# cwozny/sdr_channelizer

Hardware: AMD Instinct MI355X
Metric: input MS/s (complex) channelized (higher is better)
Workload: dtype f32; 1 GPU; cfg2: M=64 channels, 12 taps/branch, D=64, int16 I/Q (12-bit), 2^30 samples per GPU per step, frame-major complex64 out; kernel=pfb_fast<M64,P12,D64,int16>, schedule=default (4: FIR/FFT wave pairs, 8x64-frame workgroups), samples_per_gpu=1073741824, prewarm_steps=20, parallelism=single GPU

## Files before the change

### sdr_channelizer_amd/csrc/pfb_api.cpp

```cpp
#include <hip/hip_runtime.h>

#include <algorithm>
#include <cmath>
#include <cstdio>
#include <cstring>
#include <new>
#include <stdexcept>
#include <string>
#include <utility>
#include <vector>

#include "pfb_common.h"
#include "pfb_channelizer_dev.h"
#include "pfb_host.h"
#include "pfb_launch_policy.h"

using pfb::DeviceGuard;
using pfb::g_detail;
using pfb::hip_fail;

namespace {

constexpr uint32_t kStateMagic = 0x50464231u;

struct StateHeader {
  uint32_t magic, M, P, D, fmt, hist_samples, phase, reserved;
  uint64_t frame_index;
};

}

struct pfb_handle {
  int M = 0, P = 0, D = 0, off = 0;
  int fmt = 0, bit_width = 0, layout = 0;
  unsigned flags = 0;
  int device = 0;
  int num_cus = 256;
  int bps = 0;
// ... 95 lines not shown
    q.layout = PFB_LAYOUT_FRAME_MAJOR;
    q.out = static_cast<float2*>(h->d_slab);
    q.frames = std::min<long long>(sf, p.frames - f0);
    q.frame0 = p.frame0 + f0;
    q.in = static_cast<const char*>(p.in) + (size_t)f0 * h->D * h->bps;
    q.n_in = p.n_in - f0 * h->D;
    if (f0 > 0)
      q.hist = static_cast<const char*>(q.in) - (size_t)h->hist_samples * h->bps;
    HIP_TRY(h->fast->launch(q, h->stream));
    HIP_TRY(pfb::launch_transpose_slab(h->d_slab, q.frames, h->M, p.out, p.out_ld, p.out_frame0 + f0, h->out_elem, h->stream));
  }
  return PFB_OK;
}

int launch_frames(pfb_handle* h, const void* d_iq, uint64_t n, const void* hist, void* d_out, uint64_t f_begin,
                  uint64_t f_end, int64_t out_ld, int64_t out_frame0) {
  if (f_end <= f_begin) return PFB_OK;
  if (f_begin > 0) {
    if (f_begin * (uint64_t)h->D < (uint64_t)h->hist_samples) return PFB_ERR_BAD_ARG;
    const size_t skip = (size_t)f_begin * h->D * h->bps;
    hist = static_cast<const char*>(d_iq) + skip - (size_t)h->hist_samples * h->bps;
    d_iq = static_cast<const char*>(d_iq) + skip;
    n -= f_begin * (uint64_t)h->D;
    if (h->layout == PFB_LAYOUT_FRAME_MAJOR) d_out = static_cast<char*>(d_out) + (size_t)f_begin * h->M * h->out_elem;
    else out_frame0 += (int64_t)f_begin;
  }
  const uint64_t frames = f_end - f_begin;
  pfb::KernelParams p{};
  p.in = d_iq;
  p.hist = hist;
  p.out = static_cast<float2*>(d_out);
// ... 24 lines not shown
  if (prc != PFB_OK) return prc;
  if (want_fast) {
    const pfb::LaunchRequest rq{h->opt_schedule, h->opt_frames_per_block, h->opt_xcd_remap, h->opt_slab_frames,
                                h->layout == PFB_LAYOUT_CHANNEL_MAJOR, (h->flags & PFB_FLAG_MAGNITUDE) != 0, h->num_cus};
    const pfb_launch_report rep = pfb::plan_launch(h->plan, rq, frames);
    p.schedule = rep.schedule;
    p.frames_per_block = rep.frames_per_block;
    p.xcd_remap = rep.xcd_remap;
    const int cpt = h->fast->cols_per_thread;
    const int bmod = ((p.base % cpt) + cpt) % cpt;
    p.vec_ok = (bmod == 0) && (reinterpret_cast<uintptr_t>(d_iq) % (uintptr_t)(h->bps * cpt) == 0);
    if (rep.by_slabs) {
      const int rc = launch_by_slabs(h, p, (long long)rep.slab_frames);
      if (rc != PFB_OK) return rc;
    } else {
      HIP_TRY(h->fast->launch(p, h->stream));
    }
    h->last_kernel = h->fast->name;
    h->last_launch = rep;
  } else {
    HIP_TRY(pfb::launch_generic(p, h->stream));
    h->last_kernel = "pfb_generic";
    h->last_launch = pfb_launch_report{};
    h->last_launch.frames = frames;
  }
  if (ev_second) HIP_TRY(hipEventRecord(ev_second, h->stream));
  return PFB_OK;
}

int advance_state(pfb_handle* h, const void* d_iq, uint64_t n, uint64_t frames) {
  if (n > 0) {
    HIP_TRY(pfb::launch_update_history(h->d_hist[h->cur], d_iq, (long long)n, h->d_hist[h->cur ^ 1],
                                       h->hist_samples, h->bps, h->stream));
    h->cur ^= 1;
  }
  h->phase = (uint32_t)((h->phase + n) % (uint64_t)h->D);
  h->frame_index += frames;
  return PFB_OK;
}

int enqueue(pfb_handle* h, const void* d_iq, uint64_t n, void* d_out, uint64_t frames, int64_t out_ld,
            int64_t out_frame0) {
  const int rc = launch_frames(h, d_iq, n, h->d_hist[h->cur], d_out, 0, frames, out_ld, out_frame0);
  if (rc != PFB_OK) return rc;
  return advance_state(h, d_iq, n, frames);
}

int process_host(pfb_handle* h, const void* iq, uint64_t n, const pfb::StageOut& out, uint64_t chunk = 0) {
  if (chunk == 0) chunk = h->opt_host_chunk > 0 ? (uint64_t)h->opt_host_chunk : (uint64_t)1 << 24;
  chunk = ((chunk + h->D - 1) / h->D) * h->D;
  const pfb::StageSteps steps{
      chunk, chunk / h->D + 1, (size_t)h->bps, (size_t)h->M * h->out_elem,
      [h](uint64_t m) { return frames_for(h, m); },
      [h](const void* d_in, uint64_t m, void* d_out, uint64_t f, int64_t out_ld, int64_t out_row0) {
        return enqueue(h, d_in, m, d_out, f, out_ld, out_row0);
      }};
  return pfb::stage_host(h->stage, h->stream, steps, iq, n, out);
}

hipError_t make_lane_tables(const pfb_handle* h, const pfb::FastKernelInfo* f, float** taps_lane, float2** tw_lane) {
// ... 742 lines not shown
```

### sdr_channelizer_amd/csrc/pfb_common.h

```cpp
#pragma once

#include <hip/hip_runtime.h>
#include <stdint.h>

#include <new>

#include "pfb_channelizer.h"

namespace pfb {

template <class F>
static inline int abi_guard(F&& body) noexcept {
  try {
    return body();
  } catch (const std::bad_alloc&) {
    return PFB_ERR_NO_MEMORY;
  } catch (...) {
    return PFB_ERR_INTERNAL;
  }
}

struct KernelParams {
  const void* in;
  const void* hist;
// ... 9 lines not shown
  long long out_frame0;
  int base;
  int hist_samples;
  int frames_per_block;
  int vec_ok;
  int M, P, D;
  int fmt;
  int layout;
  unsigned flags;
  int nontemporal;
  int xcd_remap;
  int experiment;
  int schedule;
  int tile_waves;
  int grid_override;
};

template <int FMT> struct SampleT;
template <> struct SampleT<PFB_FMT_INT16_IQ> {
  using raw_t = uint32_t;
  static constexpr int kBytes = 4;
  static __device__ __forceinline__ void cvt(raw_t v, float& re, float& im) {
    re = (float)(int16_t)(v & 0xffffu);
    im = (float)((int32_t)v >> 16);
  }
};
template <> struct SampleT<PFB_FMT_INT8_IQ> {
  using raw_t = uint16_t;
  static constexpr int kBytes = 2;
  static __device__ __forceinline__ void cvt(raw_t v, float& re, float& im) {
// ... 77 lines not shown
```

### sdr_channelizer_amd/csrc/pfb_fast.hpp

```cpp
#pragma once

#include "pfb_fast_halo.hpp"
#include "pfb_fast_overlap.hpp"
#include "pfb_fast_pairs.hpp"
#include "pfb_fast_seg.hpp"
#include "pfb_fast_sliding.hpp"
#include "pfb_fast_teams.hpp"
#include "pfb_fast_tiles.hpp"
#include "pfb_fast_twin.hpp"

namespace pfb {

template <class K>
constexpr bool kChannelMajorOk = K::NT < 1024 && !(K::NP == 3 && K::C <= 4);

template <class K>
hipError_t launch_fast(const KernelParams& p, hipStream_t s) {
  if (p.frames <= 0) return hipSuccess;
  if (p.layout == PFB_LAYOUT_CHANNEL_MAJOR) {
    if constexpr (kChannelMajorOk<K>) {
      if constexpr (K::NT == 64) {
        if constexpr (kTileTOk<K, 4, 2>) {
          if (p.schedule == 8 || p.schedule < 0) {
            const int key = p.tile_waves * 100 + (p.schedule == 8 ? p.frames_per_block / K::C : 0);
// ... 16 lines not shown
            if (nwv == 16) return launch_tile<K, 16, true>(p, s);
          }
          return launch_tile<K, 8, true>(p, s);
        }
      }
      return launch_sliding<K, true>(p, s);
    } else {
      return hipErrorInvalidValue;
    }
  }
  if constexpr (K::NT == 64 && K::NP == 2 && !K::PINGPONG) {
    if (p.schedule == 7) {
      constexpr size_t kPair = sizeof(float2) * 2 * K::BUF;
      if (p.tile_waves == 4) return launch_pairs_sliding<K, 4, 2>(p, s);
      if constexpr (K::MIN_WAVES >= 4 && 8 * kPair <= 160 * 1024) {
        if (p.tile_waves >= 8) return launch_pairs_sliding<K, 8, 4>(p, s);
      }
      return launch_pairs_sliding<K, 6, 3>(p, s);
    }
  }
  if constexpr (kOverlapOk<K>) {
    if (p.schedule == 11) return launch_overlap<K>(p, s);
  }
  if constexpr (kTwinOk<K>) {
    if (p.schedule == 13) {
      if (p.layout != PFB_LAYOUT_FRAME_MAJOR) return hipErrorInvalidValue;
      return launch_twin<K>(p, s);
    }
  }
  if constexpr (kTeamsOk<K>) {
    if (p.schedule == 6) return launch_teams<K>(p, s);
  }
  if constexpr (K::NT == 64 && K::NP == 2 && !K::PINGPONG && K::M == 64 && K::C == 8) {
    if (p.schedule == 4) {
      const int key = p.tile_waves * 1000 + p.frames_per_block;
      if constexpr (K::FMT == PFB_FMT_INT16_IQ && K::M == 64 && K::P == 12) {
        switch (key) {
          case 4064: return launch_paired<K, 4, 64, 4>(p, s);
          case 5064: return launch_paired<K, 5, 64, 5>(p, s);
          case 8048: return launch_paired<K, 8, 48, 4>(p, s);
          case 8128: return launch_paired<K, 8, 128, 4>(p, s);
          default: break;
        }
      }
      constexpr size_t kPair = sizeof(float2) * 2 * K::BUF, kSlot = sizeof(typename SampleT<K::FMT>::raw_t) * (K::W - 1) * K::D;
      if constexpr (8 * kPair + 9 * kSlot <= 160 * 1024) {
        if (p.tile_waves == 4) return launch_paired<K, 4, 64, 2>(p, s);
        return launch_paired<K, 8, 64, 4>(p, s);
      } else {
        return launch_paired<K, 4, 64, 2>(p, s);
      }
    }
  }
  if constexpr (K::NT == 64 && K::C == 8 && !K::PINGPONG) {
    if (p.schedule == 3) {
      const int key = p.tile_waves * 1000 + p.frames_per_block;
      hipError_t r = hipErrorNotSupported;
      if (key == 8024) r = launch_shared<K, 8, 24>(p, s);
      else if (key == 8032) r = launch_shared<K, 8, 32>(p, s);
      else if (key == 8064) r = launch_shared<K, 8, 64>(p, s);
      else if (key == 4064) r = launch_shared<K, 4, 64>(p, s);
      else {
        bool done = false;
        if constexpr (K::FMT == PFB_FMT_INT16_IQ && K::M == 64 && K::P == 12) {
          switch (key) {
// ... 25 lines not shown
```

### sdr_channelizer_amd/csrc/pfb_fast_cfg.hpp

```cpp
#pragma once

#include "pfb_cplx.hpp"

namespace pfb {


template <int M_, int P_, int D_, int CPT_, int FMT_, int C_, int NP_, int R0_, int R1_, int R2_, int RS0_,
          int RS1_, int RS2_, int FS_, bool PINGPONG_, int MIN_WAVES_, bool TW_TABLE_ = false, bool WAVE_FRAMES_ = false>
struct FastCfg {
  static constexpr bool WAVE_FRAMES = WAVE_FRAMES_;
  static constexpr int M = M_, P = P_, D = D_, CPT = CPT_, FMT = FMT_, C = C_, NP = NP_;
  static constexpr int LANES = D / CPT;
  static constexpr int NT = (LANES + 63) / 64 * 64;
  static constexpr bool POW2 = (M & (M - 1)) == 0;
  static constexpr int W = M * P / D;
  static constexpr int OS = M / D;
  static constexpr int FS = FS_;
  static constexpr bool PINGPONG = PINGPONG_;
  static constexpr bool TW_TABLE = TW_TABLE_;
  static constexpr int MIN_WAVES = MIN_WAVES_;
  static constexpr int R(int i) { return i == 0 ? R0_ : i == 1 ? R1_ : R2_; }
  static constexpr int RS(int i) { return i == 0 ? RS0_ : i == 1 ? RS1_ : RS2_; }
  static constexpr int S(int i) { int s = 1; for (int j = i + 1; j < NP; ++j) s *= R(j); return s; }
  static constexpr int K(int i) { int k = 1; for (int j = 0; j < i; ++j) k *= R(j); return k; }
// ... 17 lines not shown
PFB_DEV long long xcd_remap_block(long long blk, long long nb, int mode) {
  if (mode == 1) {
    const long long q = nb >> 3, r = nb & 7, xc = blk & 7;
    return (xc < r ? xc * (q + 1) : r * (q + 1) + (xc - r) * q) + (blk >> 3);
  }
  if (mode > 1) {
    const long long G = mode, span = 8 * G, base = (blk / span) * span;
    if (base + span <= nb) {
      const long long in = blk - base;
      return base + (in & 7) * G + (in >> 3);
    }
  }
  return blk;
}

template <class K>
struct FastRows {
  using ST = SampleT<K::FMT>;
  using raw_t = typename ST::raw_t;
  static constexpr int D = K::D, CPT = K::CPT, C = K::C, NT = K::NT;

  struct alignas(sizeof(raw_t) * CPT) RawVec { raw_t v[CPT]; };

  PFB_DEV v2f cvt(raw_t r) {
    float re, im;
    ST::cvt(r, re, im);
    return (v2f){re, im};
  }

  template <bool INTERIOR>
// ... 120 lines not shown
```

### sdr_channelizer_amd/csrc/pfb_fast_core.hpp

```cpp
#pragma once

#include "pfb_fast_cfg.hpp"

namespace pfb {

template <class K, bool CM = false, bool MS = false>
struct FastKernel : FastRows<K> {
  static constexpr int M = K::M, P = K::P, D = K::D, CPT = K::CPT, C = K::C, W = K::W, OS = K::OS, NT = K::NT;
  static constexpr int NW = W - 1 + C;

  template <int I, bool FULL = false, int MAGSEL = -1>
  PFB_DEV void pass(const KernelParams& p, float2* src, float2* dst, int tid, long long f0,
                    const v2f (&tw)[2][16]) {
    float2* const p_out = p.out;
    const long long p_frames = p.frames;
    constexpr int R = K::R(I), S = K::S(I), KK = K::K(I), RS = K::RS(I);
    constexpr int IPF = M / R, ITEMS = C * IPF, ITERS = (ITEMS + NT - 1) / NT;
    constexpr bool LAST = (I == K::NP - 1);
    constexpr bool TW_REGS = (ITERS == 1) && !K::TW_TABLE;
    constexpr bool READ_BARRIER = !LAST && !K::PINGPONG && NT > 64;
    constexpr bool kMagStaged = MS && LAST;
#pragma unroll
    for (int it = 0; it < ITERS; ++it) {
      const int w = tid + it * NT;
      const bool active = (ITEMS % NT == 0) || (w < ITEMS);
      const int fc = w / IPF, item = w % IPF;
      const int kk = item / S, rest = item % S;
      v2f x[R];
      if (active) {
        const v2f* s2 = reinterpret_cast<const v2f*>(src) + fc * K::FS + item;
// ... 61 lines not shown
          const int shift = (p.flags & PFB_FLAG_FFTSHIFT) ? (M / 2) : 0;
          auto col_of = [&](int ch) {
            const int c2 = ch + shift;
            return c2 >= M ? c2 - M : c2;
          };
          auto slot = [&](auto* rowp, int k) {
            if constexpr (K::POW2) {
              auto* lo = rowp + kk + shift;
              auto* hi = rowp + kk + (M / 2 - shift);
              return (k < R / 2) ? lo + k * KK : hi + (k - R / 2) * KK;
            } else {
              return rowp + col_of(kk + k * KK);
            }
          };
          if constexpr (CM || (!K::POW2 && K::NT == 64)) {
            const bool mag = (p.flags & PFB_FLAG_MAGNITUDE) != 0;
            const long long esz = mag ? 4 : 8;
            const long long cs = CM ? p.out_ld : 1;
            int col = col_of(kk);
            char* ptr = reinterpret_cast<char*>(p_out) + ((long long)col * cs + (CM ? p.out_frame0 + f : f * M)) * esz;
            const long long step = (long long)KK * cs * esz, wrap = (long long)M * cs * esz;
#pragma unroll
            for (int k = 0; k < R; ++k) {
              v2f v = x[k];
              if (mag) {
                *reinterpret_cast<float*>(ptr) = mag_out(v.x, v.y, p.flags);
              } else {
                v = derot(v, k);
                store_c64(reinterpret_cast<float2*>(ptr), v, p.nontemporal);
              }
              asm volatile("" : "+v"(ptr) : : "memory");
              col += KK;
              ptr += step;
              if (col >= M) { col -= M; ptr -= wrap; }
            }
          } else if (MAGSEL == 1 || (MAGSEL < 0 && (p.flags & PFB_FLAG_MAGNITUDE))) {
            float* rowm = reinterpret_cast<float*>(p_out) + f0 * M + fc * M;
#pragma unroll
            for (int k = 0; k < R; ++k) *slot(rowm, k) = mag_out(x[k].x, x[k].y, p.flags);
          } else {
            float2* row = p_out + f0 * M + fc * M;
#pragma unroll
            for (int k = 0; k < R; ++k) {
              const v2f v = derot(x[k], k);
              store_c64(slot(row, k), v, p.nontemporal);
            }
          }
        }
      }
    }
  }

  PFB_DEV int tslot_frame(int col, int fc) {
    constexpr int IPF = M / K::R(K::NP - 1), NFC = IPF >= 16 ? 1 : 16 / IPF, Q = 16 / C;
    static_assert(16 % C == 0 && (IPF >= 16 || 16 % IPF == 0) && C % NFC == 0, "power-of-two chunk and lane groups");
    return fc ^ (NFC * ((col / Q) % (C / NFC)));
  }

  PFB_DEV void last_pass_transposed(const KernelParams& p, float2* slot, int tid, long long f0) {
    constexpr int I = K::NP - 1;
// ... 175 lines not shown
          for (int t = 0; t < C; ++t) {
            if (q == 0 && (j & 1)) fma_tap0_hi(acc[t], x[W - 1 + t - j][cc], k.hp[j >> 1][cc]);
            else if (q == 0) fma_tap0_lo(acc[t], x[W - 1 + t - j][cc], k.hp[j >> 1][cc]);
            else if (j & 1) fma_tap_hi(acc[t], x[W - 1 + t - j][cc], k.hp[j >> 1][cc], tok);
            else fma_tap_lo(acc[t], x[W - 1 + t - j][cc], k.hp[j >> 1][cc], tok);
          }
        }
        if (!(K::LANES < NT) || tid < K::LANES) {
#pragma unroll
          for (int t = 0; t < C; ++t)
            reinterpret_cast<v2f*>(buf)[t * K::FS + k.upos[ph][cc]] = acc[t] * k.conj_mul;
        }
      }
  }

  PFB_DEV void fft_from_lds(const KernelParams& p, const Consts& k, float2* buf, int tid, long long f0) {
    static_assert(K::NP == 2 && !K::PINGPONG, "two in-place passes");
    pass<0>(p, buf, buf, tid, f0, k.tw);
    team_sync<true>();
    pass<1>(p, buf, nullptr, tid, f0, k.tw);
  }
};

}
```

### sdr_channelizer_amd/csrc/pfb_fast_halo.hpp

```cpp
#pragma once

#include "pfb_fast_core.hpp"

namespace pfb {

template <class K>
struct HaloShare : FastKernel<K> {
  using F = FastKernel<K>;
  using typename F::raw_t; using typename F::Consts;
  using F::cvt; using F::setup; using F::fir_to_lds; using F::fft_from_lds;
  static constexpr int M = K::M, P = K::P, D = K::D, CPT = K::CPT, C = K::C, W = K::W, OS = K::OS, NT = K::NT, NW = F::NW;

  template <bool INTERIOR, int NWV, int L>
  PFB_DEV void shared_impl(const KernelParams& p, const Consts& k, float2* lds, raw_t* halo_mine,
                           const raw_t* halo_next, int wave, long long f_begin) {
    static_assert(L % C == 0 && L >= W - 1, "runs are whole chunks and at least one halo long");
    constexpr int TAIL0 = L - (W - 1);
    const int tid = threadIdx.x & 63;
    const int c0 = tid * CPT;
    const raw_t* run_ptr = static_cast<const raw_t*>(p.in) + ((f_begin - (W - 1)) * D + p.base);
    v2f x[NW][CPT];
    raw_t raw[C][CPT];
#pragma unroll
    for (int i = 0; i < W - 1; ++i) {
// ... 106 lines not shown
#pragma unroll
          for (int cc = 0; cc < CPT; ++cc) x[W - 1 + t][cc] = cvt(raw[ci % DEPTH][t][cc]);
        }
      }
      if (ci + DEPTH < NCH) fetch(ci + DEPTH);
      fir_to_lds(k, x, bufs + (ci & 1) * K::BUF, tid);
#pragma unroll
      for (int i = 0; i < W - 1; ++i)
#pragma unroll
        for (int cc = 0; cc < CPT; ++cc) x[i][cc] = x[i + C][cc];
      __syncthreads();
    }
    __syncthreads();
  }

  template <int NPAIR, int L>
  PFB_DEV void run_paired(const KernelParams& p, float2* lds_fft, raw_t* lds_halo) {
    static_assert(NT == 64, "one wave per run and role");
    static_assert(L % C == 0 && L >= W - 1, "runs are whole chunks and at least one halo long");
    constexpr int NCH = L / C;
    const int wave = threadIdx.x >> 6, tid = threadIdx.x & 63;
    const bool fir_role = wave < NPAIR;
    const int pair = fir_role ? wave : wave - NPAIR;
    long long blk = blockIdx.x;
    blk = xcd_remap_block(blk, gridDim.x, p.xcd_remap);
    const long long f_blk = blk * (long long)(NPAIR * L);
    const long long f_begin = f_blk + (long long)pair * L;
    float2* bufs = lds_fft + pair * 2 * K::BUF;
    const bool interior = p.vec_ok && ((f_blk - (W - 1)) * D + p.base >= 0) && (f_blk + NPAIR * L <= p.frames);
    if (fir_role) {
      raw_t* halo_mine = lds_halo + pair * ((W - 1) * D);
      const raw_t* halo_next = lds_halo + (pair + 1) * ((W - 1) * D);
      if (interior) paired_fir_role<true, NPAIR, L>(p, bufs, halo_mine, halo_next, pair, f_begin);
      else paired_fir_role<false, NPAIR, L>(p, bufs, halo_mine, halo_next, pair, f_begin);
    } else {
      Consts k;
      setup(p, tid, k);
      __syncthreads();
#pragma unroll
      for (int s = 0; s <= NCH; ++s) {
        if (s >= 1) fft_from_lds(p, k, bufs + ((s - 1) & 1) * K::BUF, tid, f_begin + (long long)(s - 1) * C);
        __syncthreads();
      }
    }
  }
};

template <class K, int NWV, int L>
__global__ void __launch_bounds__(64 * NWV) pfb_shared_kernel(const KernelParams p) {
  using raw_t = typename SampleT<K::FMT>::raw_t;
  __shared__ float2 lds_fft[NWV * K::LDS_ELEMS];
  __shared__ raw_t lds_halo[(NWV + 1) * (K::W - 1) * K::D];
  HaloShare<K>::template run_shared<NWV, L>(p, lds_fft, lds_halo);
}

template <class K, int NPAIR, int L, int MINW>
__global__ void __launch_bounds__(128 * NPAIR, MINW) pfb_paired_kernel(const KernelParams p) {
  using raw_t = typename SampleT<K::FMT>::raw_t;
  __shared__ float2 lds_fft[NPAIR * 2 * K::BUF];
  __shared__ raw_t lds_halo[(NPAIR + 1) * (K::W - 1) * K::D];
  HaloShare<K>::template run_paired<NPAIR, L>(p, lds_fft, lds_halo);
}

template <class K, int NPAIR, int L, int MINW>
hipError_t launch_paired(const KernelParams& p, hipStream_t s) {
  return launch_blocks(&pfb_paired_kernel<K, NPAIR, L, MINW>, blocks_for(p, (long long)NPAIR * L), 128 * NPAIR, p, s);
}

template <class K, int NWV>
constexpr bool kSharedFits = sizeof(float2) * NWV * K::LDS_ELEMS +
                                 sizeof(typename SampleT<K::FMT>::raw_t) * (NWV + 1) * (K::W - 1) * K::D <= 160 * 1024;

template <class K, int NWV, int L>
hipError_t launch_shared_impl(const KernelParams& p, hipStream_t s) {
  const unsigned extra_lds = (unsigned)((p.experiment >> 8) & 0xff) * 1024u;
  return launch_blocks(&pfb_shared_kernel<K, NWV, L>, blocks_for(p, (long long)NWV * L), 64 * NWV, p, s, extra_lds);
}

template <class K, int NWV, int L>
hipError_t launch_shared(const KernelParams& p, hipStream_t s) {
  if constexpr (kSharedFits<K, NWV>) {
// ... 10 lines not shown
```

### sdr_channelizer_amd/csrc/pfb_fast_overlap.hpp

```cpp
#pragma once

#include "pfb_fast_core.hpp"
#include <utility>

namespace pfb {

template <class K>
struct Overlap : FastKernel<K> {
  using F = FastKernel<K>;
  using typename F::raw_t; using typename F::Consts;
  using F::cvt; using F::setup;
  static constexpr int M = K::M, P = K::P, D = K::D, CPT = K::CPT, C = K::C, W = K::W, OS = K::OS, NT = K::NT, NW = F::NW;

  static constexpr int NWP = (NW + C - 1) / C * C, PERIOD = NWP / C;
  static constexpr bool kRingOk = PERIOD >= 2 && PERIOD <= 4;
  static constexpr bool kBuiltinFir = OS == 2 && CPT == 1;
  template <int PH = 0, int NX = NW>
  PFB_DEV void fir_compute(const Consts& k, const v2f (&xw)[NX][CPT], v2f (&acc)[OS][CPT][C]) {
    auto x = [&](int i) -> const v2f (&)[CPT] { return xw[(i + C * PH) % NX]; };
#pragma unroll
    for (int ph = 0; ph < OS; ++ph)
#pragma unroll
      for (int cc = 0; cc < CPT; ++cc) {
        if constexpr (kBuiltinFir) {
// ... 156 lines not shown
    setup(p, threadIdx.x, k);
    const bool interior = p.vec_ok && ((f_begin - (W - 1)) * D + p.base >= 0) && (f_last <= p.frames);
    if constexpr (kRingOk) {
      if (interior && p.frames_per_block == C * PERIOD) {
        run_overlap_ring<MAGSEL>(p, k, lds, f_begin);
        return;
      }
    }
    if (interior) run_overlap_impl<true, MAGSEL>(p, k, lds, f_begin, f_end);
    else run_overlap_impl<false, MAGSEL>(p, k, lds, f_begin, f_end);
  }
};

template <class K, bool MAG>
__global__ void __launch_bounds__(K::NT, (K::MIN_WAVES > 2 ? K::MIN_WAVES - 1 : K::MIN_WAVES)) pfb_overlap_kernel(const KernelParams p) {
  __shared__ float2 lds[2 * K::BUF];
  Overlap<K>::template run_overlap<MAG ? 1 : 0>(p, lds);
}

template <class K>
constexpr bool kOverlapOk = K::NT == 64 && K::NP == 2 && !K::PINGPONG;

template <class K>
hipError_t launch_overlap(const KernelParams& p, hipStream_t s) {
  return launch_blocks(wants_magnitude(p) ? &pfb_overlap_kernel<K, true> : &pfb_overlap_kernel<K, false>,
                       blocks_for(p, p.frames_per_block), K::NT, p, s);
}

}
```

### sdr_channelizer_amd/csrc/pfb_fast_pairs.hpp

```cpp
#pragma once

#include "pfb_fast_core.hpp"

namespace pfb {

template <class K>
struct PairSlide : FastKernel<K> {
  using F = FastKernel<K>;
  using typename F::raw_t; using typename F::Consts; using typename F::RowFetch;
  using F::cvt; using F::setup; using F::finish_rows; using F::fir_to_lds; using F::fft_from_lds;
  static constexpr int M = K::M, P = K::P, D = K::D, CPT = K::CPT, C = K::C, W = K::W, OS = K::OS, NT = K::NT, NW = F::NW;

  template <bool INTERIOR>
  PFB_DEV void pair_fir_run(const KernelParams& p, const Consts& k, float2* bufs, long long f_begin, int nch) {
    const int tid = threadIdx.x & 63;
    const int c0 = tid * CPT;
    const raw_t* run_ptr = static_cast<const raw_t*>(p.in) + ((f_begin - (W - 1)) * D + p.base);
    v2f x[NW][CPT];
    raw_t raw[C][CPT];
#pragma unroll
    for (int i = 0; i < W - 1; ++i) {
      raw_t t[CPT];
      F::template load_row<INTERIOR>(p, run_ptr, f_begin - (W - 1) + i, i, c0, t);
#pragma unroll
// ... 14 lines not shown
        if (ci + 1 < nch) {
          const long long rel = (long long)(ci + 1) * C + (W - 1);
          F::template load_rows<INTERIOR>(p, run_ptr, f_begin + (long long)(ci + 1) * C, rel, c0, raw, rf);
        }
        fir_to_lds(k, x, bufs + u * K::BUF, tid);
#pragma unroll
        for (int i = 0; i < W - 1; ++i)
#pragma unroll
          for (int cc = 0; cc < CPT; ++cc) x[i][cc] = x[i + C][cc];
        __syncthreads();
      }
    }
    __syncthreads();
  }

  template <int NPAIR>
  PFB_DEV void run_pairs_sliding(const KernelParams& p, float2* lds_fft) {
    static_assert(NT == 64 && K::NP == 2 && !K::PINGPONG, "one wave per role, two in-place passes");
    const int wave = threadIdx.x >> 6, tid = threadIdx.x & 63;
    const bool fir_role = wave < NPAIR;
    const int pair = fir_role ? wave : wave - NPAIR;
    long long blk = blockIdx.x;
    blk = xcd_remap_block(blk, gridDim.x, p.xcd_remap);
    const long long f_begin = (blk * NPAIR + pair) * (long long)p.frames_per_block;
    const int nch = p.frames_per_block / C;
    float2* bufs = lds_fft + pair * 2 * K::BUF;
    Consts k;
    setup(p, tid, k);
    if (fir_role) {
      const bool interior = p.vec_ok && ((f_begin - (W - 1)) * D + p.base >= 0) && (f_begin + p.frames_per_block <= p.frames);
      if (f_begin >= p.frames) {
        for (int s = 0; s <= nch; ++s) __syncthreads();
      } else if (interior) {
        pair_fir_run<true>(p, k, bufs, f_begin, nch);
      } else {
        pair_fir_run<false>(p, k, bufs, f_begin, nch);
      }
    } else {
#pragma unroll 1
      for (int s = 0; s <= nch; ++s) {
        if (s >= 1 && f_begin < p.frames) fft_from_lds(p, k, bufs + ((s - 1) & 1) * K::BUF, tid, f_begin + (long long)(s - 1) * C);
        __syncthreads();
      }
    }
  }
};

template <class K, int NPAIR, int MINW>
__global__ void __launch_bounds__(128 * NPAIR, MINW) pfb_pairs_sliding_kernel(const KernelParams p) {
  __shared__ float2 lds_fft[NPAIR * 2 * K::BUF];
  PairSlide<K>::template run_pairs_sliding<NPAIR>(p, lds_fft);
}

template <class K, int NPAIR, int MINW>
hipError_t launch_pairs_sliding(const KernelParams& p, hipStream_t s) {
  return launch_blocks(&pfb_pairs_sliding_kernel<K, NPAIR, MINW>, blocks_for(p, (long long)NPAIR * p.frames_per_block), 128 * NPAIR, p, s);
}

}
```

### sdr_channelizer_amd/csrc/pfb_fast_seg.hpp

```cpp
#pragma once

#include "pfb_fast_cfg.hpp"

namespace pfb {

template <class K>
struct SegKernel {
  using ST = SampleT<K::FMT>;
  using raw_t = typename ST::raw_t;
  static constexpr int M = K::M, P = K::P, D = K::D, C = K::C, W = K::W;
  static constexpr int SEG = 64 / M, CT = C * SEG, NW = W - 1 + C;
  static_assert(K::NT == 64 && K::CPT == 1 && K::OS == 1 && K::NP == 2 && K::PINGPONG && SEG >= 1, "small banks");

  PFB_DEV v2f cvt(raw_t r) {
    float re, im;
    ST::cvt(r, re, im);
    return (v2f){re, im};
  }

  template <bool INTERIOR>
  PFB_DEV raw_t load(const KernelParams& p, long long s, long long f) {
    const raw_t* in = static_cast<const raw_t*>(p.in);
    if constexpr (INTERIOR) {
      return in[s];
// ... 132 lines not shown
  template <int MAGSEL = -1, int CMSEL = -1>
  PFB_DEV void run(const KernelParams& p, float2* lds) {
    long long run = blockIdx.x;
    run = xcd_remap_block(run, gridDim.x, p.xcd_remap);
    const long long f_begin = run * p.frames_per_block;
    if (f_begin >= p.frames) return;
    const long long l_seg = p.frames_per_block / SEG;
    const bool interior = p.vec_ok && ((f_begin - (W - 1)) * D + p.base >= 0) && (f_begin + p.frames_per_block <= p.frames);
    if (interior) run_impl<true, MAGSEL, CMSEL>(p, lds, f_begin, l_seg);
    else run_impl<false, MAGSEL, CMSEL>(p, lds, f_begin, l_seg);
  }
};

template <class K, bool MAG, bool CMAJ>
__global__ void __launch_bounds__(64, K::MIN_WAVES) pfb_seg_kernel(const KernelParams p) {
  __shared__ float2 lds[2 * SegKernel<K>::CT * K::FS];
  SegKernel<K>::template run<MAG ? 1 : 0, CMAJ ? 1 : 0>(p, lds);
}

template <class K>
hipError_t launch_seg(const KernelParams& p, hipStream_t s) {
  if (p.frames <= 0) return hipSuccess;
  const bool mag = wants_magnitude(p), cm = p.layout == PFB_LAYOUT_CHANNEL_MAJOR;
  return launch_blocks(mag ? (cm ? &pfb_seg_kernel<K, true, true> : &pfb_seg_kernel<K, true, false>)
                           : (cm ? &pfb_seg_kernel<K, false, true> : &pfb_seg_kernel<K, false, false>),
                       blocks_for(p, p.frames_per_block), 64, p, s);
}

}
```

### sdr_channelizer_amd/csrc/pfb_fast_sliding.hpp

```cpp
#pragma once

#include "pfb_fast_core.hpp"

namespace pfb {

template <class K, bool CM = false, bool MS = false>
struct SlidingRun : FastKernel<K, CM, MS> {
  using F = FastKernel<K, CM, MS>;
  using typename F::raw_t; using typename F::Consts; using typename F::RowFetch;
  using F::cvt; using F::setup; using F::finish_rows;
  static constexpr int M = K::M, P = K::P, D = K::D, CPT = K::CPT, C = K::C, W = K::W, OS = K::OS, NT = K::NT, NW = F::NW;

  template <bool INTERIOR, int MAGSEL = -1>
  PFB_DEV void run_impl(const KernelParams& p, const Consts& k, float2* lds, long long f_begin, long long f_end) {
    const int tid = threadIdx.x;
    const int c0 = tid * CPT;
    const raw_t* run_ptr = static_cast<const raw_t*>(p.in) + ((f_begin - (W - 1)) * D + p.base);
    v2f x[NW][CPT];
    raw_t raw[C][CPT];
#pragma unroll
    for (int i = 0; i < W - 1; ++i) {
      raw_t t[CPT];
      F::template load_row<INTERIOR>(p, run_ptr, f_begin - (W - 1) + i, i, c0, t);
#pragma unroll
// ... 38 lines not shown
    Consts k;
    setup(p, threadIdx.x, k);
    const bool interior = p.vec_ok && ((f_begin - (W - 1)) * D + p.base >= 0) && (f_last <= p.frames);
    if (interior) run_impl<true, MAGSEL>(p, k, lds, f_begin, f_end);
    else run_impl<false, MAGSEL>(p, k, lds, f_begin, f_end);
  }
};

template <class K>
constexpr bool kMagStagedOk = K::NT == 64 && K::NP == 2 && !K::PINGPONG && K::M == 64 && K::C == 8;
template <class K>
constexpr int kMagnitudeSchedule = kMagStagedOk<K> ? (K::FMT == PFB_FMT_CF32 ? 7 : 0) : -1;

template <class K, bool CM = false, bool MS = false, int MAGSEL = -1>
__global__ void __launch_bounds__(K::NT, K::MIN_WAVES) pfb_fast_kernel(const KernelParams p) {
  __shared__ float2 lds[K::LDS_ELEMS];
  SlidingRun<K, CM, MS>::template run<MAGSEL>(p, lds);
}

template <class K, bool CM = false, bool MS = false, int MAGSEL = -1>
hipError_t launch_sliding(const KernelParams& p, hipStream_t s) {
  return launch_blocks(&pfb_fast_kernel<K, CM, MS, MAGSEL>, blocks_for(p, p.frames_per_block), K::NT, p, s);
}

}
```

### sdr_channelizer_amd/csrc/pfb_fast_teams.hpp

```cpp
#pragma once

#include "pfb_fast_core.hpp"

namespace pfb {

template <class K>
struct Teams : FastKernel<K> {
  using F = FastKernel<K>;
  using typename F::raw_t; using typename F::Consts;
  using F::cvt; using F::setup; using F::fir_to_lds;
  static constexpr int M = K::M, P = K::P, D = K::D, CPT = K::CPT, C = K::C, W = K::W, OS = K::OS, NT = K::NT, NW = F::NW;

  template <int I>
  PFB_DEV void pass_frame(const KernelParams& p, float2* fbuf, int lane, const v2f (&tw)[2][16]) {
    constexpr int R = K::R(I), S = K::S(I), KK = K::K(I), RS = K::RS(I);
    constexpr int IPF = M / R, ITERS = (IPF + 63) / 64;
    constexpr int S1 = K::S(I + 1), RS1 = K::RS(I + 1);
    static_assert(I < K::NP - 1, "the last pass (with the stores) belongs to the FIR team");
    constexpr bool TW_REGS = (ITERS == 1) && !K::TW_TABLE;
    v2f x[ITERS][R];
#pragma unroll
    for (int it = 0; it < ITERS; ++it) {
      const int item = lane + it * 64;
      const bool active = (IPF % 64 == 0) || (item < IPF);
// ... 112 lines not shown
          pass_frame<1>(p, fbuf, lane, k.tw);
          b = (b == 2) ? 0 : b + 1;
        }
        __syncthreads();
      }
    }
  }
};

template <class K>
constexpr bool kTeamsOk = !K::WAVE_FRAMES && K::NP == 3 && !K::PINGPONG && K::NT > 64 && (K::NT + 64 * K::C) <= 1024 &&
                          3 * sizeof(float2) * K::BUF <= 160 * 1024 && K::C % 2 == 0;

template <class K, bool MAG>
__global__ void __launch_bounds__(K::NT + 64 * K::C, K::MIN_WAVES) pfb_teams_kernel(const KernelParams p) {
  __shared__ float2 bufs[3 * K::BUF];
  Teams<K>::template run_teams<MAG ? 1 : 0>(p, bufs);
}

template <class K>
hipError_t launch_teams(const KernelParams& p, hipStream_t s) {
  return launch_blocks(wants_magnitude(p) ? &pfb_teams_kernel<K, true> : &pfb_teams_kernel<K, false>,
                       blocks_for(p, p.frames_per_block), K::NT + 64 * K::C, p, s);
}

}
```

### sdr_channelizer_amd/csrc/pfb_fast_tiles.hpp

```cpp
#pragma once

#include "pfb_fast_core.hpp"

namespace pfb {

template <class K, bool CM = false>
struct Tiles : FastKernel<K, CM> {
  using F = FastKernel<K, CM>;
  using typename F::raw_t; using typename F::Consts; using typename F::RowFetch;
  using F::cvt; using F::setup; using F::finish_rows; using F::tslot_frame;
  static constexpr int M = K::M, P = K::P, D = K::D, CPT = K::CPT, C = K::C, W = K::W, OS = K::OS, NT = K::NT, NW = F::NW;

  PFB_DEV void load_chunk(const KernelParams& p, long long chunk, int c0, raw_t (&raw)[NW][CPT]) {
    const long long f0 = chunk * C;
    const long long s_first = (f0 - (W - 1)) * D + p.base;
    const bool interior = p.vec_ok && s_first >= 0 && (f0 + C <= p.frames);
    const raw_t* ptr = static_cast<const raw_t*>(p.in) + s_first;
    if (interior) {
#pragma unroll
      for (int i = 0; i < NW; ++i) F::template load_row<true>(p, ptr, 0, i, c0, raw[i]);
    } else {
#pragma unroll
      for (int i = 0; i < NW; ++i) F::template load_row<false>(p, ptr, f0 - (W - 1) + i, i, c0, raw[i]);
    }
// ... 93 lines not shown
      for (int i = 0; i < IT / HALF; ++i) {
        const int e = (h * (IT / HALF) + i) * NTH + (int)threadIdx.x, col = e / RL, fr = e % RL;
        const long long f = tf0 + fr;
        if (f < p.frames) {
          const long long idx = (long long)col * p.out_ld + p.out_frame0 + f;
          if (mag) reinterpret_cast<float*>(p.out)[idx] = mag_out(v[i].x, v[i].y, p.flags);
          else store_c64(p.out + idx, v[i], p.nontemporal);
        }
      }
    }
  }
};

template <class K, int NWV, bool CM = false>
__global__ void __launch_bounds__(64 * NWV) pfb_tile_kernel(const KernelParams p) {
  __shared__ float2 lds[NWV * K::LDS_ELEMS];
  Tiles<K, CM>::template run_tile<NWV>(p, lds);
}

template <class K, int NWV, bool CM = false>
hipError_t launch_tile(const KernelParams& p, hipStream_t s) {
  return launch_blocks(&pfb_tile_kernel<K, NWV, CM>, blocks_for(p, (long long)NWV * K::C), 64 * NWV, p, s);
}

template <class K, int NWV, int CPW>
__global__ void __launch_bounds__(64 * NWV) pfb_tile_t_kernel(const KernelParams p) {
  __shared__ float2 lds[NWV * CPW * Tiles<K, true>::TSLOT];
  Tiles<K, true>::template run_tile_t<NWV, CPW>(p, lds);
}

template <class K, int NWV, int CPW>
hipError_t launch_tile_t(const KernelParams& p, hipStream_t s) {
  return launch_blocks(&pfb_tile_t_kernel<K, NWV, CPW>, blocks_for(p, (long long)NWV * CPW * K::C), 64 * NWV, p, s);
}

template <class K>
constexpr bool kTileSlotOk = 16 % K::C == 0 && ((K::M / K::R(K::NP - 1)) >= 16 || 16 % (K::M / K::R(K::NP - 1)) == 0) &&
                             K::C % ((K::M / K::R(K::NP - 1)) >= 16 ? 1 : 16 / (K::M / K::R(K::NP - 1))) == 0;

template <class K, int NWV, int CPW>
constexpr bool kTileTOk = K::NT == 64 && K::NP == 2 && !K::PINGPONG && kTileSlotOk<K> && K::M * K::C <= K::LDS_ELEMS &&
// ... 5 lines not shown
```

### sdr_channelizer_amd/csrc/pfb_fast_twin.hpp

```cpp
#pragma once

#include "pfb_fast_core.hpp"

namespace pfb {

template <class K>
struct Twin : FastKernel<K> {
  using F = FastKernel<K>;
  using typename F::raw_t; using typename F::RawVec;
  using F::cvt;
  static constexpr bool CM = false;
  static constexpr int M = K::M, P = K::P, D = K::D, CPT = K::CPT, C = K::C, W = K::W, OS = K::OS, NT = K::NT, NW = F::NW;

  template <bool MAG>
  PFB_DEV void last_pass_frame(const KernelParams& p, const float2* fbuf, int lane, long long f) {
    constexpr int I = K::NP - 1, R = K::R(I), KK = K::K(I), RS = K::RS(I);
    constexpr int IPF = M / R, ITERS = (IPF + 63) / 64;
    static_assert(K::S(I) == 1 && !CM && OS == 1, "frame-major, critically sampled");
    v2f x[ITERS][R];
#pragma unroll
    for (int it = 0; it < ITERS; ++it) {
      const int item = lane + it * 64;
      const v2f* s2 = reinterpret_cast<const v2f*>(fbuf) + ((IPF % 64 == 0) || item < IPF ? item : 0);
#pragma unroll
// ... 301 lines not shown
    };
    for (; r < nruns && r < r_lo; r += G) careful(r);
    if (r < r_hi) {
      twin_fast<MAG>(p, lds, twl, r, G, r_hi);
      r += ((r_hi - 1 - r) / G + 1) * G;
    }
    for (; r < nruns; r += G) careful(r);
  }
};

template <class K>
constexpr bool kTwinOk = K::WAVE_FRAMES && K::NP == 3 && !K::PINGPONG && K::C % (K::NT / 64) == 0 && K::D == K::M && K::CPT % 2 == 0;

template <class K, bool MAG>
__global__ void __launch_bounds__(K::NT, K::MIN_WAVES) pfb_twin_kernel(const KernelParams p) {
  __shared__ float2 lds[K::BUF + Twin<K>::TWL_ELEMS];
  Twin<K>::template run_twin<MAG>(p, lds, lds + K::BUF);
}

template <class K>
hipError_t launch_twin(const KernelParams& p, hipStream_t s) {
  long long nb = blocks_for(p, p.frames_per_block);
  if (p.grid_override > 0 && nb > p.grid_override) nb = p.grid_override;
  return launch_blocks(wants_magnitude(p) ? &pfb_twin_kernel<K, true> : &pfb_twin_kernel<K, false>, nb, K::NT, p, s);
}

}
```

### sdr_channelizer_amd/csrc/pfb_kernels.hip

```cpp
#include "pfb_channelizer_dev.h"
#include "pfb_generic_fft.hpp"
#include "pfb_table.h"

namespace pfb {


__device__ __forceinline__ void fetch_sample(const KernelParams& p, long long s, float& re, float& im) {
  const void* b;
  long long i;
  if (s >= 0) { b = p.in; i = s; } else { b = p.hist; i = p.hist_samples + s; }
  if (p.fmt == PFB_FMT_INT16_IQ) {
    SampleT<PFB_FMT_INT16_IQ>::cvt(static_cast<const uint32_t*>(b)[i], re, im);
  } else if (p.fmt == PFB_FMT_INT8_IQ) {
    SampleT<PFB_FMT_INT8_IQ>::cvt(static_cast<const uint16_t*>(b)[i], re, im);
  } else {
    SampleT<PFB_FMT_CF32>::cvt(static_cast<const float2*>(b)[i], re, im);
  }
}

__device__ __forceinline__ int bit_reverse(int v, int bits) { return (int)(__brev((unsigned)v) >> (32 - bits)); }

__global__ void __launch_bounds__(256) pfb_generic_kernel(const KernelParams p, int tile_frames, int log2m, GenericPlan plan) {
  extern __shared__ float2 sm[];
  const int M = p.M, P = p.P, D = p.D;
  const int tid = threadIdx.x, nt = blockDim.x;
  const long long f0 = (long long)blockIdx.x * tile_frames;
  const int eff_off = p.base + D - 1;
  const float im_sign = (p.flags & PFB_FLAG_CONJUGATE_INPUT) ? -1.f : 1.f;

  for (int idx = tid; idx < tile_frames * M; idx += nt) {
    const int t = idx / M, br = idx - t * M;
    const long long f = f0 + t;
    float ar = 0.f, ai = 0.f;
    if (f < p.frames) {
      for (int q = 0; q < P; ++q) {
        float xr, xi;
        fetch_sample(p, f * D + eff_off - br - (long long)M * q, xr, xi);
        const float hq = p.taps[br + M * q];
// ... 251 lines not shown
```

Measured before the change: 481,400 MS/s.

## Fuse history carry into channelizer kernels and specialize pair kernels on output mode

Block 0 of each channelizer kernel now copies the trailing history samples into the next history buffer, so the separate update-history kernel launch per step is skipped when a single launch covers the chunk. The pair and paired FIR/FFT kernels are also templated on magnitude and nontemporal selection, and interior workgroups take a FULL path with no bounds checks. This removes one launch and its dependency bubble, but adds extra work to block 0 and more kernel instantiations. The fused carry is skipped when launching by slabs.

Result: faster. 488,300 MS/s (median of 6 runs) (+1.4%).

```diff
diff --git a/sdr_channelizer_amd/csrc/pfb_api.cpp b/sdr_channelizer_amd/csrc/pfb_api.cpp
--- a/sdr_channelizer_amd/csrc/pfb_api.cpp
+++ b/sdr_channelizer_amd/csrc/pfb_api.cpp
@@ -22,6 +22,7 @@
 namespace {
 
 constexpr uint32_t kStateMagic = 0x50464231u;
+constexpr int kExpSeparateHistory = 2;
 
 struct StateHeader {
   uint32_t magic, M, P, D, fmt, hist_samples, phase, reserved;
@@ -147,7 +148,8 @@
 }
 
 int launch_frames(pfb_handle* h, const void* d_iq, uint64_t n, const void* hist, void* d_out, uint64_t f_begin,
-                  uint64_t f_end, int64_t out_ld, int64_t out_frame0) {
+                  uint64_t f_end, int64_t out_ld, int64_t out_frame0, void* hist_out = nullptr, bool* carried = nullptr) {
+  if (carried) *carried = false;
   if (f_end <= f_begin) return PFB_OK;
   if (f_begin > 0) {
     if (f_begin * (uint64_t)h->D < (uint64_t)h->hist_samples) return PFB_ERR_BAD_ARG;
@@ -202,18 +204,27 @@
       const int rc = launch_by_slabs(h, p, (long long)rep.slab_frames);
       if (rc != PFB_OK) return rc;
     } else {
+      p.hist_out = hist_out;
       HIP_TRY(h->fast->launch(p, h->stream));
+      if (carried) *carried = hist_out != nullptr;
     }
     h->last_kernel = h->fast->name;
     h->last_launch = rep;
   } else {
+    p.hist_out = hist_out;
     HIP_TRY(pfb::launch_generic(p, h->stream));
+    if (carried) *carried = hist_out != nullptr;
     h->last_kernel = "pfb_generic";
     h->last_launch = pfb_launch_report{};
     h->last_launch.frames = frames;
   }
   if (ev_second) HIP_TRY(hipEventRecord(ev_second, h->stream));
   return PFB_OK;
+}
+
+void advance_counters(pfb_handle* h, uint64_t n, uint64_t frames) {
+  h->phase = (uint32_t)((h->phase + n) % (uint64_t)h->D);
+  h->frame_index += frames;
 }
 
 int advance_state(pfb_handle* h, const void* d_iq, uint64_t n, uint64_t frames) {
@@ -222,16 +233,21 @@
                                        h->hist_samples, h->bps, h->stream));
     h->cur ^= 1;
   }
-  h->phase = (uint32_t)((h->phase + n) % (uint64_t)h->D);
-  h->frame_index += frames;
+  advance_counters(h, n, frames);
   return PFB_OK;
 }
 
 int enqueue(pfb_handle* h, const void* d_iq, uint64_t n, void* d_out, uint64_t frames, int64_t out_ld,
             int64_t out_frame0) {
-  const int rc = launch_frames(h, d_iq, n, h->d_hist[h->cur], d_out, 0, frames, out_ld, out_frame0);
+  const bool fuse = frames > 0 && n >= (uint64_t)h->hist_samples && !(h->opt_experiment & kExpSeparateHistory);
+  bool carried = false;
+  const int rc = launch_frames(h, d_iq, n, h->d_hist[h->cur], d_out, 0, frames, out_ld, out_frame0,
+                               fuse ? h->d_hist[h->cur ^ 1] : nullptr, &carried);
   if (rc != PFB_OK) return rc;
-  return advance_state(h, d_iq, n, frames);
+  if (!carried) return advance_state(h, d_iq, n, frames);
+  h->cur ^= 1;
+  advance_counters(h, n, frames);
+  return PFB_OK;
 }
 
 int process_host(pfb_handle* h, const void* iq, uint64_t n, const pfb::StageOut& out, uint64_t chunk = 0) {
diff --git a/sdr_channelizer_amd/csrc/pfb_common.h b/sdr_channelizer_amd/csrc/pfb_common.h
--- a/sdr_channelizer_amd/csrc/pfb_common.h
+++ b/sdr_channelizer_amd/csrc/pfb_common.h
@@ -47,6 +47,7 @@
   int schedule;
   int tile_waves;
   int grid_override;
+  void* hist_out = nullptr;
 };
 
 template <int FMT> struct SampleT;
diff --git a/sdr_channelizer_amd/csrc/pfb_fast.hpp b/sdr_channelizer_amd/csrc/pfb_fast.hpp
--- a/sdr_channelizer_amd/csrc/pfb_fast.hpp
+++ b/sdr_channelizer_amd/csrc/pfb_fast.hpp
@@ -54,9 +54,9 @@
       constexpr size_t kPair = sizeof(float2) * 2 * K::BUF;
       if (p.tile_waves == 4) return launch_pairs_sliding<K, 4, 2>(p, s);
       if constexpr (K::MIN_WAVES >= 4 && 8 * kPair <= 160 * 1024) {
-        if (p.tile_waves >= 8) return launch_pairs_sliding<K, 8, 4>(p, s);
+        if (p.tile_waves >= 8) return launch_pairs_sliding_roles<K, 8, 4>(p, s);
       }
-      return launch_pairs_sliding<K, 6, 3>(p, s);
+      return launch_pairs_sliding_roles<K, 6, 3>(p, s);
     }
   }
   if constexpr (kOverlapOk<K>) {
@@ -86,9 +86,9 @@
       constexpr size_t kPair = sizeof(float2) * 2 * K::BUF, kSlot = sizeof(typename SampleT<K::FMT>::raw_t) * (K::W - 1) * K::D;
       if constexpr (8 * kPair + 9 * kSlot <= 160 * 1024) {
         if (p.tile_waves == 4) return launch_paired<K, 4, 64, 2>(p, s);
-        return launch_paired<K, 8, 64, 4>(p, s);
+        return launch_paired_roles<K, 8, 64, 4>(p, s);
       } else {
-        return launch_paired<K, 4, 64, 2>(p, s);
+        return launch_paired_roles<K, 4, 64, 2>(p, s);
       }
     }
   }
diff --git a/sdr_channelizer_amd/csrc/pfb_fast_cfg.hpp b/sdr_channelizer_amd/csrc/pfb_fast_cfg.hpp
--- a/sdr_channelizer_amd/csrc/pfb_fast_cfg.hpp
+++ b/sdr_channelizer_amd/csrc/pfb_fast_cfg.hpp
@@ -55,6 +55,36 @@
   return blk;
 }
 
+template <class T>
+PFB_DEV void carry_copy(T* dst, const T* src, int count, int tid, int nt) {
+  int i = tid;
+  for (; i + 3 * nt < count; i += 4 * nt) {
+    const T a = src[i], b = src[i + nt], c = src[i + 2 * nt], d = src[i + 3 * nt];
+    dst[i] = a;
+    dst[i + nt] = b;
+    dst[i + 2 * nt] = c;
+    dst[i + 3 * nt] = d;
+  }
+  for (; i < count; i += nt) dst[i] = src[i];
+}
+
+PFB_DEV void carry_history(const KernelParams& p, int bps, int nt) {
+  if (p.hist_out == nullptr || blockIdx.x != 0) return;
+  const char* src = static_cast<const char*>(p.in) + (p.n_in - p.hist_samples) * (long long)bps;
+  char* dst = static_cast<char*>(p.hist_out);
+  const int bytes = p.hist_samples * bps;
+  const int tid = threadIdx.x;
+  int done = 0;
+  if (((reinterpret_cast<uintptr_t>(src) | reinterpret_cast<uintptr_t>(dst)) & 15) == 0) {
+    carry_copy(reinterpret_cast<uint4*>(dst), reinterpret_cast<const uint4*>(src), bytes / 16, tid, nt);
+    done = bytes / 16 * 16;
+  }
+  const int rest = (bytes - done) / bps;
+  if (bps == 2) carry_copy(reinterpret_cast<uint16_t*>(dst + done), reinterpret_cast<const uint16_t*>(src + done), rest, tid, nt);
+  else if (bps == 4) carry_copy(reinterpret_cast<uint32_t*>(dst + done), reinterpret_cast<const uint32_t*>(src + done), rest, tid, nt);
+  else carry_copy(reinterpret_cast<uint2*>(dst + done), reinterpret_cast<const uint2*>(src + done), rest, tid, nt);
+}
+
 template <class K>
 struct FastRows {
   using ST = SampleT<K::FMT>;
diff --git a/sdr_channelizer_amd/csrc/pfb_fast_core.hpp b/sdr_channelizer_amd/csrc/pfb_fast_core.hpp
--- a/sdr_channelizer_amd/csrc/pfb_fast_core.hpp
+++ b/sdr_channelizer_amd/csrc/pfb_fast_core.hpp
@@ -9,11 +9,12 @@
   static constexpr int M = K::M, P = K::P, D = K::D, CPT = K::CPT, C = K::C, W = K::W, OS = K::OS, NT = K::NT;
   static constexpr int NW = W - 1 + C;
 
-  template <int I, bool FULL = false, int MAGSEL = -1>
+  template <int I, bool FULL = false, int MAGSEL = -1, int NTSEL = -1>
   PFB_DEV void pass(const KernelParams& p, float2* src, float2* dst, int tid, long long f0,
                     const v2f (&tw)[2][16]) {
     float2* const p_out = p.out;
     const long long p_frames = p.frames;
+    const int nontemporal = NTSEL < 0 ? p.nontemporal : NTSEL;
     constexpr int R = K::R(I), S = K::S(I), KK = K::K(I), RS = K::RS(I);
     constexpr int IPF = M / R, ITEMS = C * IPF, ITERS = (ITEMS + NT - 1) / NT;
     constexpr bool LAST = (I == K::NP - 1);
@@ -105,7 +106,7 @@
             }
           };
           if constexpr (CM || (!K::POW2 && K::NT == 64)) {
-            const bool mag = (p.flags & PFB_FLAG_MAGNITUDE) != 0;
+            const bool mag = MAGSEL < 0 ? (p.flags & PFB_FLAG_MAGNITUDE) != 0 : MAGSEL == 1;
             const long long esz = mag ? 4 : 8;
             const long long cs = CM ? p.out_ld : 1;
             int col = col_of(kk);
@@ -118,7 +119,7 @@
                 *reinterpret_cast<float*>(ptr) = mag_out(v.x, v.y, p.flags);
               } else {
                 v = derot(v, k);
-                store_c64(reinterpret_cast<float2*>(ptr), v, p.nontemporal);
+                store_c64(reinterpret_cast<float2*>(ptr), v, nontemporal);
               }
               asm volatile("" : "+v"(ptr) : : "memory");
               col += KK;
@@ -134,7 +135,7 @@
 #pragma unroll
             for (int k = 0; k < R; ++k) {
               const v2f v = derot(x[k], k);
-              store_c64(slot(row, k), v, p.nontemporal);
+              store_c64(slot(row, k), v, nontemporal);
             }
           }
         }
@@ -340,11 +341,12 @@
       }
   }
 
+  template <bool FULL = false, int MAGSEL = -1, int NTSEL = -1>
   PFB_DEV void fft_from_lds(const KernelParams& p, const Consts& k, float2* buf, int tid, long long f0) {
     static_assert(K::NP == 2 && !K::PINGPONG, "two in-place passes");
     pass<0>(p, buf, buf, tid, f0, k.tw);
     team_sync<true>();
-    pass<1>(p, buf, nullptr, tid, f0, k.tw);
+    pass<1, FULL, MAGSEL, NTSEL>(p, buf, nullptr, tid, f0, k.tw);
   }
 };
 
diff --git a/sdr_channelizer_amd/csrc/pfb_fast_halo.hpp b/sdr_channelizer_amd/csrc/pfb_fast_halo.hpp
--- a/sdr_channelizer_amd/csrc/pfb_fast_halo.hpp
+++ b/sdr_channelizer_amd/csrc/pfb_fast_halo.hpp
@@ -144,7 +144,7 @@
     __syncthreads();
   }
 
-  template <int NPAIR, int L>
+  template <int NPAIR, int L, int MAGSEL = -1, int NTSEL = -1>
   PFB_DEV void run_paired(const KernelParams& p, float2* lds_fft, raw_t* lds_halo) {
     static_assert(NT == 64, "one wave per run and role");
     static_assert(L % C == 0 && L >= W - 1, "runs are whole chunks and at least one halo long");
@@ -167,10 +167,20 @@
       Consts k;
       setup(p, tid, k);
       __syncthreads();
-#pragma unroll
-      for (int s = 0; s <= NCH; ++s) {
-        if (s >= 1) fft_from_lds(p, k, bufs + ((s - 1) & 1) * K::BUF, tid, f_begin + (long long)(s - 1) * C);
-        __syncthreads();
+      if (interior) {
+#pragma unroll
+        for (int s = 0; s <= NCH; ++s) {
+          if (s >= 1)
+            F::template fft_from_lds<true, MAGSEL, NTSEL>(p, k, bufs + ((s - 1) & 1) * K::BUF, tid, f_begin + (long long)(s - 1) * C);
+          __syncthreads();
+        }
+      } else {
+#pragma unroll
+        for (int s = 0; s <= NCH; ++s) {
+          if (s >= 1)
+            F::template fft_from_lds<false, MAGSEL, NTSEL>(p, k, bufs + ((s - 1) & 1) * K::BUF, tid, f_begin + (long long)(s - 1) * C);
+          __syncthreads();
+        }
       }
     }
   }
@@ -178,23 +188,31 @@
 
 template <class K, int NWV, int L>
 __global__ void __launch_bounds__(64 * NWV) pfb_shared_kernel(const KernelParams p) {
+  carry_history(p, SampleT<K::FMT>::kBytes, 64 * NWV);
   using raw_t = typename SampleT<K::FMT>::raw_t;
   __shared__ float2 lds_fft[NWV * K::LDS_ELEMS];
   __shared__ raw_t lds_halo[(NWV + 1) * (K::W - 1) * K::D];
   HaloShare<K>::template run_shared<NWV, L>(p, lds_fft, lds_halo);
 }
 
-template <class K, int NPAIR, int L, int MINW>
+template <class K, int NPAIR, int L, int MINW, int MAGSEL = -1, int NTSEL = -1>
 __global__ void __launch_bounds__(128 * NPAIR, MINW) pfb_paired_kernel(const KernelParams p) {
+  carry_history(p, SampleT<K::FMT>::kBytes, 128 * NPAIR);
   using raw_t = typename SampleT<K::FMT>::raw_t;
   __shared__ float2 lds_fft[NPAIR * 2 * K::BUF];
   __shared__ raw_t lds_halo[(NPAIR + 1) * (K::W - 1) * K::D];
-  HaloShare<K>::template run_paired<NPAIR, L>(p, lds_fft, lds_halo);
+  HaloShare<K>::template run_paired<NPAIR, L, MAGSEL, NTSEL>(p, lds_fft, lds_halo);
+}
+
+template <class K, int NPAIR, int L, int MINW, int MAGSEL = -1, int NTSEL = -1>
+hipError_t launch_paired(const KernelParams& p, hipStream_t s) {
+  return launch_blocks(&pfb_paired_kernel<K, NPAIR, L, MINW, MAGSEL, NTSEL>, blocks_for(p, (long long)NPAIR * L), 128 * NPAIR, p, s);
 }
 
 template <class K, int NPAIR, int L, int MINW>
-hipError_t launch_paired(const KernelParams& p, hipStream_t s) {
-  return launch_blocks(&pfb_paired_kernel<K, NPAIR, L, MINW>, blocks_for(p, (long long)NPAIR * L), 128 * NPAIR, p, s);
+hipError_t launch_paired_roles(const KernelParams& p, hipStream_t s) {
+  if (wants_magnitude(p)) return launch_paired<K, NPAIR, L, MINW, 1, 0>(p, s);
+  return p.nontemporal ? launch_paired<K, NPAIR, L, MINW, 0, 1>(p, s) : launch_paired<K, NPAIR, L, MINW, 0, 0>(p, s);
 }
 
 template <class K, int NWV>
diff --git a/sdr_channelizer_amd/csrc/pfb_fast_overlap.hpp b/sdr_channelizer_amd/csrc/pfb_fast_overlap.hpp
--- a/sdr_channelizer_amd/csrc/pfb_fast_overlap.hpp
+++ b/sdr_channelizer_amd/csrc/pfb_fast_overlap.hpp
@@ -194,6 +194,7 @@
 
 template <class K, bool MAG>
 __global__ void __launch_bounds__(K::NT, (K::MIN_WAVES > 2 ? K::MIN_WAVES - 1 : K::MIN_WAVES)) pfb_overlap_kernel(const KernelParams p) {
+  carry_history(p, SampleT<K::FMT>::kBytes, K::NT);
   __shared__ float2 lds[2 * K::BUF];
   Overlap<K>::template run_overlap<MAG ? 1 : 0>(p, lds);
 }
diff --git a/sdr_channelizer_amd/csrc/pfb_fast_pairs.hpp b/sdr_channelizer_amd/csrc/pfb_fast_pairs.hpp
--- a/sdr_channelizer_amd/csrc/pfb_fast_pairs.hpp
+++ b/sdr_channelizer_amd/csrc/pfb_fast_pairs.hpp
@@ -52,7 +52,7 @@
     __syncthreads();
   }
 
-  template <int NPAIR>
+  template <int NPAIR, int MAGSEL = -1, int NTSEL = -1>
   PFB_DEV void run_pairs_sliding(const KernelParams& p, float2* lds_fft) {
     static_assert(NT == 64 && K::NP == 2 && !K::PINGPONG, "one wave per role, two in-place passes");
     const int wave = threadIdx.x >> 6, tid = threadIdx.x & 63;
@@ -74,25 +74,40 @@
       } else {
         pair_fir_run<false>(p, k, bufs, f_begin, nch);
       }
+    } else if (f_begin + p.frames_per_block <= p.frames) {
+#pragma unroll 1
+      for (int s = 0; s <= nch; ++s) {
+        if (s >= 1)
+          F::template fft_from_lds<true, MAGSEL, NTSEL>(p, k, bufs + ((s - 1) & 1) * K::BUF, tid, f_begin + (long long)(s - 1) * C);
+        __syncthreads();
+      }
     } else {
 #pragma unroll 1
       for (int s = 0; s <= nch; ++s) {
-        if (s >= 1 && f_begin < p.frames) fft_from_lds(p, k, bufs + ((s - 1) & 1) * K::BUF, tid, f_begin + (long long)(s - 1) * C);
+        if (s >= 1 && f_begin < p.frames)
+          F::template fft_from_lds<false, MAGSEL, NTSEL>(p, k, bufs + ((s - 1) & 1) * K::BUF, tid, f_begin + (long long)(s - 1) * C);
         __syncthreads();
       }
     }
   }
 };
 
-template <class K, int NPAIR, int MINW>
+template <class K, int NPAIR, int MINW, int MAGSEL = -1, int NTSEL = -1>
 __global__ void __launch_bounds__(128 * NPAIR, MINW) pfb_pairs_sliding_kernel(const KernelParams p) {
+  carry_history(p, SampleT<K::FMT>::kBytes, 128 * NPAIR);
   __shared__ float2 lds_fft[NPAIR * 2 * K::BUF];
-  PairSlide<K>::template run_pairs_sliding<NPAIR>(p, lds_fft);
+  PairSlide<K>::template run_pairs_sliding<NPAIR, MAGSEL, NTSEL>(p, lds_fft);
+}
+
+template <class K, int NPAIR, int MINW, int MAGSEL = -1, int NTSEL = -1>
+hipError_t launch_pairs_sliding(const KernelParams& p, hipStream_t s) {
+  return launch_blocks(&pfb_pairs_sliding_kernel<K, NPAIR, MINW, MAGSEL, NTSEL>, blocks_for(p, (long long)NPAIR * p.frames_per_block), 128 * NPAIR, p, s);
 }
 
 template <class K, int NPAIR, int MINW>
-hipError_t launch_pairs_sliding(const KernelParams& p, hipStream_t s) {
-  return launch_blocks(&pfb_pairs_sliding_kernel<K, NPAIR, MINW>, blocks_for(p, (long long)NPAIR * p.frames_per_block), 128 * NPAIR, p, s);
+hipError_t launch_pairs_sliding_roles(const KernelParams& p, hipStream_t s) {
+  if (wants_magnitude(p)) return launch_pairs_sliding<K, NPAIR, MINW, 1, 0>(p, s);
+  return p.nontemporal ? launch_pairs_sliding<K, NPAIR, MINW, 0, 1>(p, s) : launch_pairs_sliding<K, NPAIR, MINW, 0, 0>(p, s);
 }
 
 }
diff --git a/sdr_channelizer_amd/csrc/pfb_fast_seg.hpp b/sdr_channelizer_amd/csrc/pfb_fast_seg.hpp
--- a/sdr_channelizer_amd/csrc/pfb_fast_seg.hpp
+++ b/sdr_channelizer_amd/csrc/pfb_fast_seg.hpp
@@ -170,6 +170,7 @@
 
 template <class K, bool MAG, bool CMAJ>
 __global__ void __launch_bounds__(64, K::MIN_WAVES) pfb_seg_kernel(const KernelParams p) {
+  carry_history(p, SampleT<K::FMT>::kBytes, 64);
   __shared__ float2 lds[2 * SegKernel<K>::CT * K::FS];
   SegKernel<K>::template run<MAG ? 1 : 0, CMAJ ? 1 : 0>(p, lds);
 }
diff --git a/sdr_channelizer_amd/csrc/pfb_fast_sliding.hpp b/sdr_channelizer_amd/csrc/pfb_fast_sliding.hpp
--- a/sdr_channelizer_amd/csrc/pfb_fast_sliding.hpp
+++ b/sdr_channelizer_amd/csrc/pfb_fast_sliding.hpp
@@ -76,6 +76,7 @@
 
 template <class K, bool CM = false, bool MS = false, int MAGSEL = -1>
 __global__ void __launch_bounds__(K::NT, K::MIN_WAVES) pfb_fast_kernel(const KernelParams p) {
+  carry_history(p, SampleT<K::FMT>::kBytes, K::NT);
   __shared__ float2 lds[K::LDS_ELEMS];
   SlidingRun<K, CM, MS>::template run<MAGSEL>(p, lds);
 }
diff --git a/sdr_channelizer_amd/csrc/pfb_fast_teams.hpp b/sdr_channelizer_amd/csrc/pfb_fast_teams.hpp
--- a/sdr_channelizer_amd/csrc/pfb_fast_teams.hpp
+++ b/sdr_channelizer_amd/csrc/pfb_fast_teams.hpp
@@ -150,6 +150,7 @@
 
 template <class K, bool MAG>
 __global__ void __launch_bounds__(K::NT + 64 * K::C, K::MIN_WAVES) pfb_teams_kernel(const KernelParams p) {
+  carry_history(p, SampleT<K::FMT>::kBytes, K::NT + 64 * K::C);
   __shared__ float2 bufs[3 * K::BUF];
   Teams<K>::template run_teams<MAG ? 1 : 0>(p, bufs);
 }
diff --git a/sdr_channelizer_amd/csrc/pfb_fast_tiles.hpp b/sdr_channelizer_amd/csrc/pfb_fast_tiles.hpp
--- a/sdr_channelizer_amd/csrc/pfb_fast_tiles.hpp
+++ b/sdr_channelizer_amd/csrc/pfb_fast_tiles.hpp
@@ -131,6 +131,7 @@
 
 template <class K, int NWV, bool CM = false>
 __global__ void __launch_bounds__(64 * NWV) pfb_tile_kernel(const KernelParams p) {
+  carry_history(p, SampleT<K::FMT>::kBytes, 64 * NWV);
   __shared__ float2 lds[NWV * K::LDS_ELEMS];
   Tiles<K, CM>::template run_tile<NWV>(p, lds);
 }
@@ -142,6 +143,7 @@
 
 template <class K, int NWV, int CPW>
 __global__ void __launch_bounds__(64 * NWV) pfb_tile_t_kernel(const KernelParams p) {
+  carry_history(p, SampleT<K::FMT>::kBytes, 64 * NWV);
   __shared__ float2 lds[NWV * CPW * Tiles<K, true>::TSLOT];
   Tiles<K, true>::template run_tile_t<NWV, CPW>(p, lds);
 }
diff --git a/sdr_channelizer_amd/csrc/pfb_fast_twin.hpp b/sdr_channelizer_amd/csrc/pfb_fast_twin.hpp
--- a/sdr_channelizer_amd/csrc/pfb_fast_twin.hpp
+++ b/sdr_channelizer_amd/csrc/pfb_fast_twin.hpp
@@ -339,6 +339,7 @@
 
 template <class K, bool MAG>
 __global__ void __launch_bounds__(K::NT, K::MIN_WAVES) pfb_twin_kernel(const KernelParams p) {
+  carry_history(p, SampleT<K::FMT>::kBytes, K::NT);
   __shared__ float2 lds[K::BUF + Twin<K>::TWL_ELEMS];
   Twin<K>::template run_twin<MAG>(p, lds, lds + K::BUF);
 }
diff --git a/sdr_channelizer_amd/csrc/pfb_kernels.hip b/sdr_channelizer_amd/csrc/pfb_kernels.hip
--- a/sdr_channelizer_amd/csrc/pfb_kernels.hip
+++ b/sdr_channelizer_amd/csrc/pfb_kernels.hip
@@ -22,6 +22,7 @@
 
 __global__ void __launch_bounds__(256) pfb_generic_kernel(const KernelParams p, int tile_frames, int log2m, GenericPlan plan) {
   extern __shared__ float2 sm[];
+  carry_history(p, p.fmt == PFB_FMT_INT8_IQ ? 2 : (p.fmt == PFB_FMT_INT16_IQ ? 4 : 8), 256);
   const int M = p.M, P = p.P, D = p.D;
   const int tid = threadIdx.x, nt = blockDim.x;
   const long long f0 = (long long)blockIdx.x * tile_frames;
```
